# Wil-Lee/NN_BVH

Measured on AMD Instinct MI355X. Metric: Mray/s (closest-hit + any-hit), higher is better.
Workload: dtype f32; 1 GPU; crown, 1000x1400: one wavefront pass of 8 spp per step (8 spp per GPU-film) — primary, bounce-1 and bounce-2 closest-hit, shadow any-hit towards the light quads (batches pre-generated, hence independent: ONE launch; the dependent form is dependent_step), rays in --ray-order tile (a caller-side order the reference's integrator does not form: ray_order_probe), RecordShadowRayResult + RGBFilm::AddSam; sample_sets=4, geometry=procedural stand-in for crown (3548192 tris; data/crown.npz absent), tree=sah, triangles=3548192, nodes=7032259, rays_primary=11200000, rays_bounce=7410327, rays_bounce2=4392209, parallelism=tile-sharded x1, BVH replicated, film all-gather after the pass

## Files before the change

nn_bvh_amd/csrc/bvh_trace.hip:

```cpp
#include <hip/hip_runtime.h>
#include <stdint.h>

#include "bvh_trace.h"
#include "anim_math.h"
#include "spawn_math.h"
#include "trace_math.h"

namespace nnbvh {

constexpr int kDone = (int)0x80000000;
constexpr int kReturn = (int)0x80000001;
constexpr int kEnter = (int)0x80000002;

#ifndef NNBVH_MINW_CLOSEST
#define NNBVH_MINW_CLOSEST 6
#endif
#ifndef NNBVH_MINW_ANY
#define NNBVH_MINW_ANY 6
#endif
#ifndef NNBVH_LEAN_EXTRA_WAVES
#define NNBVH_LEAN_EXTRA_WAVES 2
#endif
#ifndef NNBVH_MINW_ALPHA
#define NNBVH_MINW_ALPHA 5
#endif
#ifndef NNBVH_MINW_ALPHA_PATCH
#define NNBVH_MINW_ALPHA_PATCH 3
#endif
#ifndef NNBVH_ANIM_ENTER_WEIGHT
#define NNBVH_ANIM_ENTER_WEIGHT 8
#endif
template <typename T>
__device__ __forceinline__ T pick_batch(const T (&a)[kMaxFusedBatches], int b) {
    static_assert(kMaxFusedBatches == 4, "written out for four batches");
    return b == 0 ? a[0] : (b == 1 ? a[1] : (b == 2 ? a[2] : a[3]));
}

template <int MODE, int W, int INST, int PATCH, int ALPHA = 0, int SOA = 0, int HOSTC = 0>
__global__ __launch_bounds__(kBlockThreads, (INST ? 1 : (ALPHA ? (ALPHA == 2 ? NNBVH_MINW_ALPHA_PATCH : NNBVH_MINW_ALPHA) : ((MODE == 0 || MODE == 3) ? NNBVH_MINW_CLOSEST : NNBVH_MINW_ANY) + (PATCH ? 0 : NNBVH_LEAN_EXTRA_WAVES))))
void trace_kernel(TraceParams p) {
    static_assert(PATCH || !INST, "two-level scenes need the ray direction");
    static_assert(PATCH || !ALPHA, "the alpha test hashes the ray direction");
    static_assert(!HOSTC || (PATCH && (MODE == 0 || MODE == 2 || (MODE == 3 && !ALPHA && W == 8)) && !SOA),
                  "candidate mode: general instances of modes 0 / 2 / 3");
    __shared__ float s_stack[kBlockThreads / 64][W][2][64];
    constexpr bool kLean = !PATCH && !INST;
    constexpr int kColdRi = 0, kColdD = 1, kColdHit = kLean ? 0 : (PATCH ? 4 : 1),
                  kColdHost = kColdHit + ((MODE == 0 || MODE == 3) ? 4 : 0);
    constexpr int kColdBase = kColdHost + (kLean ? 0 : 1);
    constexpr int kSaveO = kColdBase, kSaveInv = kColdBase + 3, kSaveShear = kColdBase + 6,
                  kSaveKz = kColdBase + 9, kSaveTmax = kColdBase + 10, kSaveD = kColdBase + 11,
                  kResume = kColdBase + 14, kCurInst = kColdBase + 15, kHitInst = kColdBase + 16,
                  kInnerHit = kColdBase + 17, kColdTime = kColdBase + 18, kPendSlot = kColdBase + 19;
    constexpr int kColdFields = kColdBase + (INST ? 20 : 0);
    __shared__ float s_cold[kBlockThreads / 64][kColdFields > 0 ? kColdFields : 1][64];

    const int lane = threadIdx.x & 63;
    const int wave = threadIdx.x >> 6;
    const int gtid = blockIdx.x * kBlockThreads + threadIdx.x;
    float(*stk)[2][64] = s_stack[wave];
    float(*cold)[64] = s_cold[wave];
    int riReg = -1;
    if (!kLean) cold[kColdRi][lane] = __int_as_float(-1);
    const long spillStride = (long)gridDim.x * kBlockThreads;

    int q = 0;
    if (p.nQueues > 1) {
        unsigned xcc;
        asm volatile("s_getreg_b32 %0, hwreg(HW_REG_XCC_ID)" : "=s"(xcc));
        q = (int)(xcc & 0xf) % p.nQueues;
    }
    int queuesTried = 0;
    int curBatch = 0;
    long nRays = p.n;
    if (p.nDev) {
        const long nd = (long)*p.nDev;
        nRays = nd < 0 ? 0 : (nd < nRays ? nd : nRays);
    }

#ifdef NNBVH_STATS
    unsigned long long st[16] = {0, 0, 0, 0, 0, 0, 0, 0, 0, 0, 0, 0, 0, 0, 0, 0};
    unsigned long long stPrev = __builtin_amdgcn_s_memtime();
    int stKind = 2;
#endif
    RayState r;
    RayMasks masks = {0ull, 0ull, 0ull, 0ull, 0ull, 0ull};
    float tMax = 0.0f;
    int visited = 0, tests = 0;
    int cur = kDone, sp = 0, base = 0;
    int floor = -1;
    bool found = false;
    bool exhausted = false;

    auto pop_entry = [&](int &ref, float &key) {
        --sp;
        ref = __float_as_int(stk[sp & (W - 1)][0][lane]);
        key = stk[sp & (W - 1)][1][lane];
        asm volatile("" : "+v"(ref), "+v"(key));
        if (sp < base) {
            const uint2 e = p.spill[(long)sp * spillStride + gtid];
            base = sp;
            ref = (int)e.x;
            key = __uint_as_float(e.y);
            asm volatile("" : "+v"(ref), "+v"(key));
        }
        if (MODE != 2) visited += 1;
    };
    auto pop_next = [&]() -> int {
        const int lowest = (INST && floor > 0) ? floor : 0;
        const int none = (INST && floor >= 0) ? kReturn : kDone;
        if (sp <= lowest) return none;
        int ref;
        float key;
        pop_entry(ref, key);
        if (key < tMax) return ref;
        while (sp > lowest) {
            pop_entry(ref, key);
            if (key < tMax) return ref;
        }
        return none;
    };

    auto enter_instance = [&](int slot, unsigned flags, float4 s0, float4 s1, float4 s2) {
        const float4 s3 = p.prims[slot + 3], s4 = p.prims[slot + 4], s5 = p.prims[slot + 5];
        const V3 dOuter = {cold[kColdD][lane], cold[kColdD + 1][lane], cold[kColdD + 2][lane]};
        cold[kSaveO][lane] = r.o.x;
        cold[kSaveO + 1][lane] = r.o.y;
        cold[kSaveO + 2][lane] = r.o.z;
        cold[kSaveInv][lane] = r.inv.x;
        cold[kSaveInv + 1][lane] = r.inv.y;
        cold[kSaveInv + 2][lane] = r.inv.z;
        cold[kSaveShear][lane] = r.sx;
        cold[kSaveShear + 1][lane] = r.sy;
        cold[kSaveShear + 2][lane] = r.sz;
        cold[kSaveKz][lane] = __int_as_float(r.kz);
        cold[kSaveTmax][lane] = tMax;
        cold[kSaveD][lane] = dOuter.x;
        cold[kSaveD + 1][lane] = dOuter.y;
        cold[kSaveD + 2][lane] = dOuter.z;
        cold[kResume][lane] = __int_as_float((flags & kPrimLast) ? kDone : ~(slot + 6));
        cold[kCurInst][lane] = __int_as_float(__float_as_int(s0.w) + 1);
        cold[kInnerHit][lane] = 0.0f;
        V3 oIn, dIn;
        float4 m0 = s2, m1 = s3, m2 = s4;
        if (INST == 2 && (flags & kPrimAnimated) && p.anim)
            anim_inverse_rows(p.anim + (long)kAnimStride * __float_as_int(s0.w), cold[kColdTime][lane], m0, m1, m2);
        apply_inverse_ray(m0, m1, m2, r.o, dOuter, tMax, oIn, dIn);
        r.o = oIn;
        cold[kColdD][lane] = dIn.x;
        cold[kColdD + 1][lane] = dIn.y;
        cold[kColdD + 2][lane] = dIn.z;
        r.inv = {1.0f / dIn.x, 1.0f / dIn.y, 1.0f / dIn.z};
        ray_shear(r, dIn);
        floor = sp;
        if (MODE != 2) visited += 1;
        float tEntry;
        const bool rootHit =
            slab_partial(s0.x, s0.y, s0.z, s1.x, s1.y, s1.z, r, tEntry) && (tEntry < tMax);
        cur = rootHit ? __float_as_int(s5.x) : kReturn;
    };

    auto leave_instance = [&]() {
        const bool innerHit = cold[kInnerHit][lane] != 0.0f;
        r.o = {cold[kSaveO][lane], cold[kSaveO + 1][lane], cold[kSaveO + 2][lane]};
        r.inv = {cold[kSaveInv][lane], cold[kSaveInv + 1][lane], cold[kSaveInv + 2][lane]};
        r.sx = cold[kSaveShear][lane];
        r.sy = cold[kSaveShear + 1][lane];
        r.sz = cold[kSaveShear + 2][lane];
        r.kz = __float_as_int(cold[kSaveKz][lane]);
        cold[kColdD][lane] = cold[kSaveD][lane];
        cold[kColdD + 1][lane] = cold[kSaveD + 1][lane];
        cold[kColdD + 2][lane] = cold[kSaveD + 2][lane];
        if (!innerHit) tMax = cold[kSaveTmax][lane];
        cold[kCurInst][lane] = 0.0f;
        floor = -1;
        const int resume = __float_as_int(cold[kResume][lane]);
        cur = (resume == kDone) ? pop_next() : resume;
    };

    auto prim_math = [&](const int slot, const float4 s0, const float4 s1, const float4 s2) {
        const unsigned flags = __float_as_uint(s1.w);
        if (INST && (flags & kPrimInstance)) {
            if (INST == 2 && NNBVH_ANIM_ENTER_WEIGHT > 0 && (flags & kPrimAnimated) && p.anim) {
                cold[kPendSlot][lane] = __int_as_float(slot);
                cur = kEnter;
            } else {
                enter_instance(slot, flags, s0, s1, s2);
            }
        } else if (!kLean && (flags & kPrimHost)) {
            if constexpr (HOSTC) {
                const int c = __float_as_int(cold[kColdHost][lane]);
                if (c >= 0) {
                    long ray = __float_as_int(cold[kColdRi][lane]);
                    int cap = p.hcCap;
                    int32_t *hcPrim = p.hcPrim, *hcInst = p.hcInst;
                    if constexpr (MODE == 3) {
                        const int b = (int)(ray >> kFusedIndexBits);
                        ray &= (1 << kFusedIndexBits) - 1;
                        cap = pick_batch(p.bHcCap, b);
                        hcPrim = pick_batch(p.bHcPrim, b);
                        hcInst = pick_batch(p.bHcInst, b);
                    }
                    if (c < cap) {
                        const long at = ray * cap + c;
                        hcPrim[at] = __float_as_int(s0.w);
                        hcInst[at] = INST ? __float_as_int(cold[kCurInst][lane]) : 0;
                    }
                    cold[kColdHost][lane] = __int_as_float(c < cap ? c + 1 : -1);
                }
            } else {
                cold[kColdHost][lane] = 1.0f;
            }
            cur = (flags & kPrimLast) ? pop_next() : ~(slot + 3);
        } else {
            tests += 1;
            bool hit;
            float x0, x1, x2, th;
            int next;
            if (!PATCH || !(flags & kPrimPatch)) {
                hit = triangle_test(r, tMax, (flags & kPrimDegenerate) != 0,
                                    {s0.x, s0.y, s0.z}, {s1.x, s1.y, s1.z},
                                    {s2.x, s2.y, s2.z}, x0, x1, x2, th, kLean ? &masks : nullptr);
                next = slot + ((ALPHA && (flags & kPrimSmooth)) ? 6 : 3);
                if (ALPHA && hit && (flags & kPrimAlpha)) {
                    const float a = s2.w;
                    if (a < 1) {
                        const V3 rd = {cold[kColdD][lane], cold[kColdD + 1][lane],
                                       cold[kColdD + 2][lane]};
                        const float u = (a <= 0) ? 1.f : hash_float_6f(r.o, rd);
                        if (u > a) {
                            hit = false;
                            RayState rn = r;
                            if (flags & kPrimSmooth) {
                                const float4 m0 = p.prims[slot + 3], m1 = p.prims[slot + 4], m2 = p.prims[slot + 5];
                                rn.o = alpha_retrace_origin({s0.x, s0.y, s0.z}, {s1.x, s1.y, s1.z}, {s2.x, s2.y, s2.z}, x0,
                                                            x1, x2, (flags & kPrimFlipN) != 0, rd, true, {m0.x, m0.y, m0.z},
                                                            {m1.x, m1.y, m1.z}, {m2.x, m2.y, m2.z});
                            } else {
                                rn.o = alpha_retrace_origin({s0.x, s0.y, s0.z}, {s1.x, s1.y, s1.z},
                                                            {s2.x, s2.y, s2.z}, x0, x1, x2,
                                                            (flags & kPrimFlipN) != 0, rd);
                            }
                            tests += 1;
                            float y0, y1, y2, tn;
                            if (triangle_test(rn, tMax - th, (flags & kPrimDegenerate) != 0,
                                              {s0.x, s0.y, s0.z}, {s1.x, s1.y, s1.z},
                                              {s2.x, s2.y, s2.z}, y0, y1, y2, tn))
                                cold[kColdHost][lane] = HOSTC ? __int_as_float(-2) : 1.0f;
                        }
                    }
                }
            } else {
                const float4 s3 = p.prims[slot + 3];
                x2 = 0.0f;
                const V3 rd = {cold[PATCH ? kColdD : 0][lane], cold[PATCH ? kColdD + 1 : 0][lane],
                               cold[PATCH ? kColdD + 2 : 0][lane]};
                next = slot + 4 + ((ALPHA == 2 && (flags & kPrimSmooth)) ? 4 : 0) + ((ALPHA == 2 && (flags & kPrimUV)) ? 2 : 0);
                if constexpr (ALPHA == 2) {
                    constexpr int kAlphaPatchDepth = 3;
                    const float a = (flags & kPrimAlpha) ? s2.w : 1.0f;
                    RayState rn = r;
                    float tm = tMax, t0 = 0.0f, t1 = 0.0f, t2 = 0.0f;
                    int k = 0;
                    for (;;) {
                        hit = patch_test(rn, rd, tm, {s0.x, s0.y, s0.z}, {s1.x, s1.y, s1.z}, {s2.x, s2.y, s2.z},
                                         {s3.x, s3.y, s3.z}, x0, x1, th);
                        if (!hit || !(a < 1)) break;
                        const float u = (a <= 0) ? 1.f : hash_float_6f(rn.o, rd);
                        if (!(u > a)) break;
                        if (k == kAlphaPatchDepth) {
                            hit = false;
                            cold[kColdHost][lane] = HOSTC ? __int_as_float(-2) : 1.0f;
                            break;
                        }
                        if (k == 0) t0 = th;
                        else if (k == 1) t1 = th;
                        else t2 = th;
                        ++k;
                        rn.o = patch_retrace_origin({s0.x, s0.y, s0.z}, {s1.x, s1.y, s1.z}, {s2.x, s2.y, s2.z},
                                                    {s3.x, s3.y, s3.z}, x0, x1, (flags & kPrimFlipN) != 0, rd,
                                                    (flags & kPrimSmooth) != 0, (flags & kPrimUV) != 0,
                                                    p.prims + slot + 4);
                        tm = tm - th;
                        tests += 1;
                    }
                    if (hit && k > 0) {
                        if (k == 3) th = th + t2;
                        if (k >= 2) th = th + t1;
                        th = th + t0;
                    }
                } else {
                    hit = patch_test(r, rd, tMax, {s0.x, s0.y, s0.z}, {s1.x, s1.y, s1.z},
                                     {s2.x, s2.y, s2.z}, {s3.x, s3.y, s3.z}, x0, x1, th);
                }
            }
            bool closestLane = MODE == 0;
            if (MODE == 3 && hit)
                closestLane = !((p.anyMask >> ((kLean ? riReg : __float_as_int(cold[kColdRi][lane])) >> kFusedIndexBits)) & 1u);
            if (hit) {
                if (closestLane) {
                    cold[kColdHit][lane] = s0.w;
                    cold[kColdHit + 1][lane] = x0;
                    cold[kColdHit + 2][lane] = x1;
                    cold[kColdHit + 3][lane] = x2;
                    tMax = th;
                    if (INST) {
                        cold[kHitInst][lane] = cold[kCurInst][lane];
                        cold[kInnerHit][lane] = 1.0f;
                    }
                    if constexpr (HOSTC && MODE == 0) {
                        const int c = __float_as_int(cold[kColdHost][lane]);
                        if (c > 0) p.hcBefore[__float_as_int(cold[kColdRi][lane])] = c;
                    }
                    if constexpr (HOSTC && MODE == 3) {
                        const int c = __float_as_int(cold[kColdHost][lane]);
                        if (c > 0) {
                            const int tag = __float_as_int(cold[kColdRi][lane]);
                            pick_batch(p.bHcBefore, tag >> kFusedIndexBits)[tag & ((1 << kFusedIndexBits) - 1)] = c;
                        }
                    }
                } else {
                    found = true;
                }
            }
            if (MODE != 0 && found) cur = kDone;
            else if (flags & kPrimLast) cur = pop_next();
            else cur = ~next;
        }
    };

    auto interior_math = [&](const float4 q0, const float4 q1, const float4 q2, const float4 q3) {
        const int ref0 = __float_as_int(q3.x), ref1 = __float_as_int(q3.y);
        const int axis = __float_as_int(q3.z);
        const bool swap = ((r.kz >> axis) & 1) != 0;
        const float k0 = kLean ? slab_entry_key(q0.x, q0.y, q0.z, q0.w, q1.x, q1.y, r, masks)
                               : slab_entry_key(q0.x, q0.y, q0.z, q0.w, q1.x, q1.y, r);
        const float k1 = kLean ? slab_entry_key(q1.z, q1.w, q2.x, q2.y, q2.z, q2.w, r, masks)
                               : slab_entry_key(q1.z, q1.w, q2.x, q2.y, q2.z, q2.w, r);
        const int nearRef = swap ? ref1 : ref0, farRef = swap ? ref0 : ref1;
        const float nearT = swap ? k1 : k0, farT = swap ? k0 : k1;
        visited += 1;
        const bool doPush = (MODE == 1) || (farT < __builtin_inff());
        if (doPush && sp - base == W - 1) {
            uint2 e;
            e.x = __float_as_uint(stk[base & (W - 1)][0][lane]);
            e.y = __float_as_uint(stk[base & (W - 1)][1][lane]);
            p.spill[(long)base * spillStride + gtid] = e;
            ++base;
        }
        stk[sp & (W - 1)][0][lane] = __int_as_float(farRef);
        stk[sp & (W - 1)][1][lane] = farT;
        sp += doPush ? 1 : 0;
        if (MODE == 0 || MODE == 3) visited += doPush ? 0 : 1;
        cur = nearT < tMax ? nearRef : pop_next();
    };
    auto interior_step = [&]() {
#ifdef NNBVH_STATS
        st[14] += 1;
        st[15] += __popcll(__ballot(cur >= 0));
#endif
        if (cur >= 0) {
            const float4 *rec = kLean ? reinterpret_cast<const float4 *>(reinterpret_cast<const char *>(p.wide) + ((unsigned)cur << 6))
                                      : p.wide + 4 * (long)cur;
            const float4 q3 = rec[3];
            const float4 q0 = rec[0], q1 = rec[1], q2 = rec[2];
            interior_math(q0, q1, q2, q3);
        }
    };

    for (;;) {
#ifdef NNBVH_STATS
        {
            const unsigned long long now = __builtin_amdgcn_s_memtime();
            st[10 + stKind] += now - stPrev;
            stPrev = now;
        }
#endif
        const bool isInt = cur >= 0;
        const bool isIdle = cur == kDone;
        const int nInt = __popcll(__ballot(isInt));
        const unsigned long long idleMask = __ballot(isIdle);
        const int nIdle = __popcll(idleMask);
        const int nEnter = (INST == 2 && NNBVH_ANIM_ENTER_WEIGHT > 0) ? __popcll(__ballot(cur == kEnter)) : 0;
        const int nPrim = 64 - nInt - nIdle - nEnter;

        const int sI = nInt * 16, sP = nPrim * p.primWeight;
        const int sR = exhausted ? 0 : nIdle * p.refillWeight;
#ifdef NNBVH_STATS
        unsigned long long &stTrips = (nIdle == 64 || (sR > sI && sR > sP)) ? st[4]
                                      : ((sP > sI || nInt == 0) ? st[2] : st[0]);
        (&stTrips)[0] += 1;
        (&stTrips)[1] += (nIdle == 64 || (sR > sI && sR > sP)) ? nIdle
                         : ((sP > sI || nInt == 0) ? nPrim : nInt);
        stKind = (&stTrips == &st[4]) ? 2 : ((&stTrips == &st[2]) ? 1 : 0);
        if (&stTrips == &st[0]) {
            st[6] += nInt;
            st[7] += nPrim;
            st[8] += nIdle;
        }
#endif
        if (nIdle == 64 || (sR > sI && sR > sP)) {
            const int ri = isIdle ? (kLean ? riReg : __float_as_int(cold[kColdRi][lane])) : -1;
            if constexpr (MODE == 3 && HOSTC) {
                if (ri >= 0) {
                    const int b = ri >> kFusedIndexBits;
                    const long idx = ri & ((1 << kFusedIndexBits) - 1);
                    void *outp = pick_batch(p.bOut, b);
                    const int c = __float_as_int(cold[kColdHost][lane]);
                    if (pick_batch(p.bHcCap, b) > 0) pick_batch(p.bHcCount, b)[idx] = c;
                    if ((p.anyMask >> b) & 1u) {
                        reinterpret_cast<uint8_t *>(outp)[idx] = found ? 1 : (c != 0 ? 2 : 0);
                    } else {
                        float4 h0, h1;
                        h0.x = cold[kColdHit][lane];
                        h0.y = tMax;
                        h0.z = cold[kColdHit + 1][lane];
                        h0.w = cold[kColdHit + 2][lane];
                        h1.x = cold[kColdHit + 3][lane];
                        h1.y = __int_as_float(visited);
                        h1.z = __int_as_float(tests);
                        h1.w = INST ? cold[kHitInst][lane] : 0.0f;
                        if (c < 0) h1.w = __int_as_float(-1);
                        float4 *out = reinterpret_cast<float4 *>(outp) + 2 * idx;
                        out[0] = h0;
                        out[1] = h1;
                    }
                }
            } else if (MODE == 3 && ri >= 0) {
                const int b = ri >> kFusedIndexBits;
                const long idx = ri & ((1 << kFusedIndexBits) - 1);
                void *outp = b == 0 ? p.bOut[0] : (b == 1 ? p.bOut[1] : (b == 2 ? p.bOut[2] : p.bOut[3]));
                const bool needHost = !kLean && p.hasHostPrims && cold[kColdHost][lane] != 0.0f;
                if ((p.anyMask >> b) & 1u) {
                    reinterpret_cast<uint8_t *>(outp)[idx] = found ? 1 : (needHost ? 2 : 0);
                } else {
                    float4 h0, h1;
                    h0.x = cold[kColdHit][lane];
                    h0.y = tMax;
                    h0.z = cold[kColdHit + 1][lane];
                    h0.w = cold[kColdHit + 2][lane];
                    h1.x = cold[kColdHit + 3][lane];
                    h1.y = __int_as_float(visited);
                    h1.z = __int_as_float(tests);
                    h1.w = INST ? cold[kHitInst][lane] : 0.0f;
                    if (needHost) h1.w = __int_as_float(-1);
                    float4 *out = reinterpret_cast<float4 *>(outp) + 2 * idx;
                    out[0] = h0;
                    out[1] = h1;
                }
            } else if (ri >= 0) {
                if (MODE == 0) {
                    float4 h0, h1;
                    h0.x = cold[kColdHit][lane];
                    h0.y = tMax;
                    h0.z = cold[kColdHit + 1][lane];
                    h0.w = cold[kColdHit + 2][lane];
                    h1.x = cold[kColdHit + 3][lane];
                    h1.y = __int_as_float(visited);
                    h1.z = __int_as_float(tests);
                    h1.w = INST ? cold[kHitInst][lane] : 0.0f;
                    if constexpr (HOSTC) {
                        const int c = __float_as_int(cold[kColdHost][lane]);
                        if (c < 0) h1.w = __int_as_float(-1);
                        p.hcCount[ri] = c;
                    } else if (!kLean && p.hasHostPrims && cold[kColdHost][lane] != 0.0f) {
                        h1.w = __int_as_float(-1);
                    }
                    float4 *out = reinterpret_cast<float4 *>(p.hits) + 2 * (long)ri;
                    out[0] = h0;
                    out[1] = h1;
                } else {
                    bool needHost;
                    if constexpr (HOSTC) {
                        const int c = __float_as_int(cold[kColdHost][lane]);
                        needHost = c != 0;
                        p.hcCount[ri] = c;
                    } else {
                        needHost = !kLean && p.hasHostPrims && cold[kColdHost][lane] != 0.0f;
                    }
                    p.occluded[ri] = found ? 1 : (needHost ? 2 : 0);
                    if (MODE == 1) {
                        if (p.visitedOut) p.visitedOut[ri] = visited;
                        if (p.testsOut) p.testsOut[ri] = tests;
                    }
                }
            }
            int newRi = -1;
            if (exhausted) break;
            long start = 0;
            for (;;) {
                if (MODE == 3) {
                    nRays = p.bN[curBatch];
                    if (const int32_t *nd = p.bNDev[curBatch]) {
                        const long v = *nd;
                        nRays = v < 0 ? 0 : (v < nRays ? v : nRays);
                    }
                }
                static_assert(kMaxQueues == 8, "queue ranges are computed with a shift by 3");
                const int qShift = p.nQueues > 1 ? 3 : 0;
                const long qBegin = (nRays * q) >> qShift, qEnd = (nRays * (q + 1)) >> qShift;
                unsigned got = 0;
                if (lane == 0)
                    got = atomicAdd(&p.queue[((MODE == 3 ? curBatch * p.nQueues : 0) + q) * kQueueStrideWords],
                                    (unsigned)nIdle);
                got = __builtin_amdgcn_readfirstlane(got);
                start = qBegin + (long)got;
                if (start < qEnd) {
                    const int rank = __builtin_amdgcn_mbcnt_hi(
                        (unsigned)(idleMask >> 32),
                        __builtin_amdgcn_mbcnt_lo((unsigned)idleMask, 0u));
                    if (isIdle && start + rank < qEnd) newRi = (int)(start + rank);
                    break;
                }
                if (++queuesTried >= p.nQueues) {
                    if (MODE == 3 && curBatch + 1 < p.nBatches) {
                        ++curBatch;
                        queuesTried = 0;
                        continue;
                    }
                    exhausted = true;
                    break;
                }
                q = (q + 1 == p.nQueues) ? 0 : q + 1;
            }
            if (isIdle) {
                const int tag = (MODE == 3 && newRi >= 0) ? (newRi | (curBatch << kFusedIndexBits)) : newRi;
                if (kLean) riReg = tag;
                else cold[kColdRi][lane] = __int_as_float(tag);
            }
            if (newRi >= 0) {
                const nnbvh_ray *batchRays = MODE == 3 ? p.bRays[curBatch] : p.rays;
                float4 r0, r1;
                if (!SOA || batchRays) {
                    const float4 *in = reinterpret_cast<const float4 *>(batchRays) + 2 * (long)newRi;
                    r0 = in[0];
                    r1 = in[1];
                } else {
                    const nnbvh_ray_soa &q = MODE == 3 ? p.bSoa[curBatch] : p.soa;
                    r0 = {q.ox[newRi], q.oy[newRi], q.oz[newRi], q.tmax ? q.tmax[newRi] : __builtin_inff()};
                    r1 = {q.dx[newRi], q.dy[newRi], q.dz[newRi], q.time ? q.time[newRi] : 0.0f};
                }
                r.o = {r0.x, r0.y, r0.z};
                tMax = r0.w;
                const V3 d = {r1.x, r1.y, r1.z};
                if (PATCH) {
                    cold[kColdD][lane] = d.x;
                    cold[kColdD + 1][lane] = d.y;
                    cold[kColdD + 2][lane] = d.z;
                }
                r.inv = {1.0f / d.x, 1.0f / d.y, 1.0f / d.z};
                ray_shear(r, d);
                if (MODE == 0 || MODE == 3) {
                    cold[kColdHit][lane] = __int_as_float(-1);
                    cold[kColdHit + 1][lane] = 0.0f;
                    cold[kColdHit + 2][lane] = 0.0f;
                    cold[kColdHit + 3][lane] = 0.0f;
                }
                if (INST) {
                    cold[kHitInst][lane] = 0.0f;
                    cold[kCurInst][lane] = 0.0f;
                    cold[kColdTime][lane] = r1.w;
                    floor = -1;
                }
                if (!kLean && (HOSTC || p.hasHostPrims)) cold[kColdHost][lane] = 0.0f;
                visited = 1;
                tests = 0;
                found = false;
                sp = base = 0;
                float tEntry;
                const bool rootHit =
                    slab_partial(p.rootMin[0], p.rootMin[1], p.rootMin[2], p.rootMax[0],
                                 p.rootMax[1], p.rootMax[2], r, tEntry) &&
                    (tEntry < tMax);
                cur = rootHit ? p.rootRef : kDone;
            }
            if (kLean) masks = ray_masks(r);
            continue;
        }

        if (INST == 2 && NNBVH_ANIM_ENTER_WEIGHT > 0 && nEnter > 0 &&
            ((nInt == 0 && nPrim == 0) || (nEnter * NNBVH_ANIM_ENTER_WEIGHT > sI && nEnter * NNBVH_ANIM_ENTER_WEIGHT > sP))) {
            if (cur == kEnter) {
                const int slot = __float_as_int(cold[kPendSlot][lane]);
                const float4 s0 = p.prims[slot], s1 = p.prims[slot + 1], s2 = p.prims[slot + 2];
                enter_instance(slot, __float_as_uint(s1.w), s0, s1, s2);
            }
            continue;
        }

        if (sP > sI || nInt == 0) {
            const int nPrep = (MODE == 3) ? 1 : p.primRepeat;
            int prep = 0;
            do {
            if (cur < 0 && cur != kDone) {
                if (INST && cur == kReturn) leave_instance();
                if (cur < 0 && cur != kDone && cur != kReturn && (INST != 2 || cur != kEnter)) {
                    const int slot = ~cur;
                    const float4 *pr = kLean ? reinterpret_cast<const float4 *>(reinterpret_cast<const char *>(p.prims) + ((unsigned)slot << 4))
                                             : p.prims + slot;
                    float4 s0 = pr[0], s1 = pr[1], s2 = pr[2];
                    asm volatile("" : "+v"(s0.x), "+v"(s0.y), "+v"(s0.z), "+v"(s0.w), "+v"(s1.x), "+v"(s1.y),
                                      "+v"(s1.z), "+v"(s1.w), "+v"(s2.x), "+v"(s2.y), "+v"(s2.z), "+v"(s2.w));
                    prim_math(slot, s0, s1, s2);
                }
            }
            } while (++prep < nPrep && __ballot(cur < 0 && cur != kDone) != 0ull);
        } else {
            if (MODE == 3) {
                interior_step();
                if (p.intRepeat > 1 && __ballot(cur >= 0) != 0ull) {
                    interior_step();
                    if (p.intRepeat > 2 && __ballot(cur >= 0) != 0ull) {
                        interior_step();
                        for (int rep = 3; rep < p.intRepeat && __ballot(cur >= 0) != 0ull; ++rep) interior_step();
                    }
                }
            } else {
            int rep = 0;
            do {
                interior_step();
            } while (++rep < p.intRepeat && __ballot(cur >= 0) != 0ull);
            }
        }
    }
#ifdef NNBVH_STATS
    if (lane == 0 && p.stats)
        for (int k = 0; k < 16; ++k) atomicAdd(&p.stats[k], st[k]);
#endif
}

template <int MODE, int W, int INST, int PATCH, int ALPHA = 0, int SOA = 0, int HOSTC = 0>
static hipError_t launch_one(const TraceParams &p, int blocks, hipStream_t stream, int *occupancy) {
    if (occupancy) {
        return hipOccupancyMaxActiveBlocksPerMultiprocessor(
            occupancy, trace_kernel<MODE, W, INST, PATCH, ALPHA, SOA, HOSTC>, kBlockThreads, 0);
    }
    hipLaunchKernelGGL((trace_kernel<MODE, W, INST, PATCH, ALPHA, SOA, HOSTC>), dim3((unsigned)blocks),
                       dim3(kBlockThreads), 0, stream, p);
    return hipGetLastError();
}

template <int MODE, int ALPHA, int HOSTC>
static hipError_t launch_inst(const TraceParams &p, int instanced, int blocks, hipStream_t stream, int *occupancy) {
    if (!instanced) return launch_one<MODE, 8, 0, 1, ALPHA, 0, HOSTC>(p, blocks, stream, occupancy);
    return p.anim ? launch_one<MODE, 8, 2, 1, ALPHA, 0, HOSTC>(p, blocks, stream, occupancy)
                  : launch_one<MODE, 8, 1, 1, ALPHA, 0, HOSTC>(p, blocks, stream, occupancy);
}
template <int MODE, int HOSTC>
static hipError_t launch_general(const TraceParams &p, int instanced, int patches, int blocks, hipStream_t stream,
                                 int *occupancy) {
    if (patches & 4) return launch_inst<MODE, 2, HOSTC>(p, instanced, blocks, stream, occupancy);
    if (patches & 2) return launch_inst<MODE, 1, HOSTC>(p, instanced, blocks, stream, occupancy);
    return launch_inst<MODE, 0, HOSTC>(p, instanced, blocks, stream, occupancy);
}

static hipError_t launch_fused(const TraceParams &p, int window, int instanced, int patches, int blocks,
                               hipStream_t stream, int *occupancy) {
    if (window != 8 || (patches & 2)) return hipErrorInvalidValue;
    if (p.hcCap > 0) {
        if (instanced) return p.anim ? launch_one<3, 8, 2, 1, 0, 0, 1>(p, blocks, stream, occupancy)
                                     : launch_one<3, 8, 1, 1, 0, 0, 1>(p, blocks, stream, occupancy);
        return launch_one<3, 8, 0, 1, 0, 0, 1>(p, blocks, stream, occupancy);
    }
    if (instanced) return p.anim ? launch_one<3, 8, 2, 1>(p, blocks, stream, occupancy)
                                 : launch_one<3, 8, 1, 1>(p, blocks, stream, occupancy);
    bool soa = false;
    for (int b = 0; b < p.nBatches; ++b) soa = soa || !p.bRays[b];
    if (!patches && !p.hasHostPrims && p.fits32)
        return soa ? launch_one<3, 8, 0, 0, 0, 1>(p, blocks, stream, occupancy) : launch_one<3, 8, 0, 0>(p, blocks, stream, occupancy);
    if (soa) return hipErrorInvalidValue;
    return launch_one<3, 8, 0, 1>(p, blocks, stream, occupancy);
}

template <int MODE>
static hipError_t launch_mode(const TraceParams &p, int window, int instanced, int patches, int blocks,
                              hipStream_t stream, int *occupancy) {
    if constexpr (MODE == 0 || MODE == 2) {
        if (p.hcCap > 0) return launch_general<MODE, 1>(p, instanced, patches, blocks, stream, occupancy);
    }
    if (instanced || (patches & 6)) return launch_general<MODE, 0>(p, instanced, patches, blocks, stream, occupancy);
    const bool soa = !p.rays && !occupancy;
    if (!patches && !p.hasHostPrims && p.fits32 && window == 8 && !instanced) {
        if (soa && MODE != 1) return launch_one<MODE == 1 ? 0 : MODE, 8, 0, 0, 0, 1>(p, blocks, stream, occupancy);
        if (!soa) return launch_one<MODE, 8, 0, 0>(p, blocks, stream, occupancy);
    }
    if (soa) return hipErrorInvalidValue;
    switch (window) {
    case 4: return launch_one<MODE, 4, 0, 1>(p, blocks, stream, occupancy);
    case 8: return launch_one<MODE, 8, 0, 1>(p, blocks, stream, occupancy);
    case 16: return launch_one<MODE, 16, 0, 1>(p, blocks, stream, occupancy);
    default: return hipErrorInvalidValue;
    }
}

__global__ void zero_queue_kernel(unsigned *queue, int words) {
    for (int i = threadIdx.x; i < words; i += blockDim.x) queue[i] = 0u;
}
hipError_t launch_zero_queue(unsigned *queue, int words, hipStream_t stream) {
    hipLaunchKernelGGL(zero_queue_kernel, dim3(1), dim3(256), 0, stream, queue, words);
    return hipGetLastError();
}

__global__ void zero_words_kernel(int32_t *words, long n) {
    for (long i = (long)blockIdx.x * blockDim.x + threadIdx.x; i < n; i += (long)gridDim.x * blockDim.x) words[i] = 0;
}
hipError_t launch_zero_words(int32_t *words, long n, int maxBlocks, hipStream_t stream) {
    long blocks = (n + 255) / 256;
    blocks = blocks < 1 ? 1 : (blocks < maxBlocks ? blocks : maxBlocks);
    hipLaunchKernelGGL(zero_words_kernel, dim3((unsigned)blocks), dim3(256), 0, stream, words, n);
    return hipGetLastError();
}

hipError_t launch_trace(int mode, const TraceParams &p, int window, int instanced, int patches, int blocks,
                        hipStream_t stream, int *occupancy) {
    switch (mode) {
    case 0: return launch_mode<0>(p, window, instanced, patches, blocks, stream, occupancy);
    case 1: return launch_mode<1>(p, window, instanced, patches, blocks, stream, occupancy);
    case 2: return launch_mode<2>(p, window, instanced, patches, blocks, stream, occupancy);
    case 3: return launch_fused(p, window, instanced, patches, blocks, stream, occupancy);
    default: return hipErrorInvalidValue;
    }
}

}
```

nn_bvh_amd/csrc/trace_math.h:

```cpp
#pragma once
#include <hip/hip_runtime.h>
#include <stdint.h>

namespace nnbvh {

#define DEV static __device__ __forceinline__

DEV constexpr float gamma_f(int n) {
    return ((float)n * 0x1p-24f) / (1.0f - (float)n * 0x1p-24f);
}

DEV float dop(float a, float b, float c, float d) {
    float cd = c * d;
    float diff = __builtin_fmaf(a, b, -cd);
    float err = __builtin_fmaf(-c, d, cd);
    return diff + err;
}

DEV float fmax3(float a, float b, float c) {
    return __builtin_fmaxf(__builtin_fmaxf(a, b), c);
}
DEV float max3(float a, float b, float c) {
    float m = a;
    if (m < b) m = b;
    if (m < c) m = c;
    return m;
}

struct V3 {
    float x, y, z;
};
DEV V3 cross(V3 v, V3 w) {
    return {dop(v.y, w.z, v.z, w.y), dop(v.z, w.x, v.x, w.z), dop(v.x, w.y, v.y, w.x)};
}
DEV float dot(V3 v, V3 w) { return v.x * w.x + v.y * w.y + v.z * w.z; }
DEV float len2(V3 v) { return v.x * v.x + v.y * v.y + v.z * v.z; }
DEV V3 sub(V3 a, V3 b) { return {a.x - b.x, a.y - b.y, a.z - b.z}; }
DEV float maxabs(V3 v) { return max3(__builtin_fabsf(v.x), __builtin_fabsf(v.y), __builtin_fabsf(v.z)); }
DEV float sel3(V3 v, int k) { return k == 0 ? v.x : (k == 1 ? v.y : v.z); }

struct RayState {
    V3 o, inv;
    float sx, sy, sz;
    int kz;
};

DEV void ray_shear(RayState &r, V3 d) {
    float ax = __builtin_fabsf(d.x), ay = __builtin_fabsf(d.y), az = __builtin_fabsf(d.z);
    int kz = (ax > ay) ? ((ax > az) ? 0 : 2) : ((ay > az) ? 1 : 2);
    int kx = kz + 1;
    if (kx == 3) kx = 0;
    int ky = kx + 1;
    if (ky == 3) ky = 0;
    float dx = kx == 0 ? d.x : (kx == 1 ? d.y : d.z);
    float dy = ky == 0 ? d.x : (ky == 1 ? d.y : d.z);
    float dz = kz == 0 ? d.x : (kz == 1 ? d.y : d.z);
    r.sx = -dx / dz;
    r.sy = -dy / dz;
    r.sz = 1.0f / dz;
    r.kz = (kz << 8) | (r.inv.x < 0.0f ? 1 : 0) | (r.inv.y < 0.0f ? 2 : 0) | (r.inv.z < 0.0f ? 4 : 0);
}

struct RayMasks {
    unsigned long long negX, negY, negZ;
    unsigned long long k0, k1, k2;
};
DEV RayMasks ray_masks(const RayState &r) {
    const int kz = r.kz >> 8;
    return {__ballot(r.inv.x < 0.0f), __ballot(r.inv.y < 0.0f), __ballot(r.inv.z < 0.0f),
            __ballot(kz == 0), __ballot(kz == 1), __ballot(kz == 2)};
}
DEV float sel_m(unsigned long long m, float a, float b) {
    float out;
    asm("v_cndmask_b32_e64 %0, %2, %1, %3" : "=v"(out) : "v"(a), "v"(b), "s"(m));
    return out;
}

DEV bool slab_partial(float mnx, float mny, float mnz, float mxx, float mxy, float mxz,
                      const RayState &r, float &tEntry) {
    constexpr float widen = 1.0f + 2.0f * gamma_f(3);
    float tMin = (((r.inv.x < 0.0f) ? mxx : mnx) - r.o.x) * r.inv.x;
    float tMax = (((r.inv.x < 0.0f) ? mnx : mxx) - r.o.x) * r.inv.x;
    float tyMin = (((r.inv.y < 0.0f) ? mxy : mny) - r.o.y) * r.inv.y;
    float tyMax = (((r.inv.y < 0.0f) ? mny : mxy) - r.o.y) * r.inv.y;
    tMax *= widen;
    tyMax *= widen;
    const bool out1 = (tMin > tyMax) | (tyMin > tMax);
    tMin = (tyMin > tMin) ? tyMin : tMin;
    tMax = (tyMax < tMax) ? tyMax : tMax;
    float tzMin = (((r.inv.z < 0.0f) ? mxz : mnz) - r.o.z) * r.inv.z;
    float tzMax = (((r.inv.z < 0.0f) ? mnz : mxz) - r.o.z) * r.inv.z;
    tzMax *= widen;
    const bool out2 = (tMin > tzMax) | (tzMin > tMax);
    tMin = (tzMin > tMin) ? tzMin : tMin;
    tMax = (tzMax < tMax) ? tzMax : tMax;
    tEntry = tMin;
    return !(out1 | out2) & (tMax > 0.0f);
}

DEV float slab_entry_key(float mnx, float mny, float mnz, float mxx, float mxy, float mxz, const RayState &r) {
    constexpr float widen = 1.0f + 2.0f * gamma_f(3);
    const float ax = (((r.inv.x < 0.0f) ? mxx : mnx) - r.o.x) * r.inv.x;
    const float bx = (((r.inv.x < 0.0f) ? mnx : mxx) - r.o.x) * r.inv.x;
    const float ay = (((r.inv.y < 0.0f) ? mxy : mny) - r.o.y) * r.inv.y;
    const float by = (((r.inv.y < 0.0f) ? mny : mxy) - r.o.y) * r.inv.y;
    const float az = (((r.inv.z < 0.0f) ? mxz : mnz) - r.o.z) * r.inv.z;
    const float bz = (((r.inv.z < 0.0f) ? mnz : mxz) - r.o.z) * r.inv.z;
    const float a = __builtin_fmaxf(__builtin_fmaxf(ax, ay), az);
    const float b = __builtin_fminf(__builtin_fminf(bx, by), bz) * widen;
    const bool ok = !__builtin_isunordered(ax, bx) & (a <= b) & (b > 0.0f);
    return ok ? a : __builtin_inff();
}

DEV float slab_entry_key(float mnx, float mny, float mnz, float mxx, float mxy, float mxz, const RayState &r,
                         const RayMasks &m) {
    constexpr float widen = 1.0f + 2.0f * gamma_f(3);
    const float ax = (sel_m(m.negX, mxx, mnx) - r.o.x) * r.inv.x;
    const float bx = (sel_m(m.negX, mnx, mxx) - r.o.x) * r.inv.x;
    const float ay = (sel_m(m.negY, mxy, mny) - r.o.y) * r.inv.y;
    const float by = (sel_m(m.negY, mny, mxy) - r.o.y) * r.inv.y;
    const float az = (sel_m(m.negZ, mxz, mnz) - r.o.z) * r.inv.z;
    const float bz = (sel_m(m.negZ, mnz, mxz) - r.o.z) * r.inv.z;
    const float a = __builtin_fmaxf(__builtin_fmaxf(ax, ay), az);
    const float b = __builtin_fminf(__builtin_fminf(bx, by), bz) * widen;
    const bool ok = !__builtin_isunordered(ax, bx) & (a <= b) & (b > 0.0f);
    return ok ? a : __builtin_inff();
}

DEV bool triangle_test(const RayState &r, float tMax, bool degenerate, V3 p0, V3 p1, V3 p2,
                       float &b0, float &b1, float &b2, float &tHit, const RayMasks *m = nullptr) {
    if (degenerate) return false;
    V3 a = sub(p0, r.o), b = sub(p1, r.o), c = sub(p2, r.o);
    float p0x, p0y, p0z, p1x, p1y, p1z, p2x, p2y, p2z;
    if (m) {
        auto px = [&](V3 v) { return sel_m(m->k2, v.x, sel_m(m->k0, v.y, v.z)); };
        auto py = [&](V3 v) { return sel_m(m->k1, v.x, sel_m(m->k2, v.y, v.z)); };
        auto pz = [&](V3 v) { return sel_m(m->k0, v.x, sel_m(m->k1, v.y, v.z)); };
        p0x = px(a), p0y = py(a), p0z = pz(a);
        p1x = px(b), p1y = py(b), p1z = pz(b);
        p2x = px(c), p2y = py(c), p2z = pz(c);
    } else {
        const int kz = r.kz >> 8;
        int kx = kz + 1;
        if (kx == 3) kx = 0;
        int ky = kx + 1;
        if (ky == 3) ky = 0;
        p0x = sel3(a, kx), p0y = sel3(a, ky), p0z = sel3(a, kz);
        p1x = sel3(b, kx), p1y = sel3(b, ky), p1z = sel3(b, kz);
        p2x = sel3(c, kx), p2y = sel3(c, ky), p2z = sel3(c, kz);
    }
    const float sx = r.sx, sy = r.sy, sz = r.sz;
    p0x += sx * p0z;
    p0y += sy * p0z;
    p1x += sx * p1z;
    p1y += sy * p1z;
    p2x += sx * p2z;
    p2y += sy * p2z;
    float e0 = dop(p1x, p2y, p1y, p2x);
    float e1 = dop(p2x, p0y, p2y, p0x);
    float e2 = dop(p0x, p1y, p0y, p1x);
    if (e0 == 0.0f || e1 == 0.0f || e2 == 0.0f) {
        double p2txp1ty = (double)p2x * (double)p1y;
        double p2typ1tx = (double)p2y * (double)p1x;
        e0 = (float)(p2typ1tx - p2txp1ty);
        double p0txp2ty = (double)p0x * (double)p2y;
        double p0typ2tx = (double)p0y * (double)p2x;
        e1 = (float)(p0typ2tx - p0txp2ty);
        double p1txp0ty = (double)p1x * (double)p0y;
        double p1typ0tx = (double)p1y * (double)p0x;
        e2 = (float)(p1typ0tx - p1txp0ty);
    }
    if ((e0 < 0 || e1 < 0 || e2 < 0) && (e0 > 0 || e1 > 0 || e2 > 0)) return false;
    float det = e0 + e1 + e2;
    if (det == 0) return false;
    p0z *= sz;
    p1z *= sz;
    p2z *= sz;
    float tScaled = e0 * p0z + e1 * p1z + e2 * p2z;
    if (det < 0 && (tScaled >= 0 || tScaled < tMax * det)) return false;
    else if (det > 0 && (tScaled <= 0 || tScaled > tMax * det)) return false;
    float invDet = 1.0f / det;
    float t = tScaled * invDet;
    const bool firstIsNan = __builtin_isunordered(p0z, p0x) | __builtin_isunordered(p0y, e0);
    float maxZt = fmax3(__builtin_fabsf(p0z), __builtin_fabsf(p1z), __builtin_fabsf(p2z));
    float deltaZ = gamma_f(3) * maxZt;
    float maxXt = fmax3(__builtin_fabsf(p0x), __builtin_fabsf(p1x), __builtin_fabsf(p2x));
    float maxYt = fmax3(__builtin_fabsf(p0y), __builtin_fabsf(p1y), __builtin_fabsf(p2y));
    float deltaX = gamma_f(5) * (maxXt + maxZt);
    float deltaY = gamma_f(5) * (maxYt + maxZt);
    float deltaE = 2.0f * (gamma_f(2) * maxXt * maxYt + deltaY * maxXt + deltaX * maxYt);
    float maxE = fmax3(__builtin_fabsf(e0), __builtin_fabsf(e1), __builtin_fabsf(e2));
    float deltaT = 3.0f * (gamma_f(3) * maxE * maxZt + deltaE * maxZt + deltaZ * maxE) *
                   __builtin_fabsf(invDet);
    if (!firstIsNan & (t <= deltaT)) return false;
    b0 = e0 * invDet;
    b1 = e1 * invDet;
    b2 = e2 * invDet;
    tHit = t;
    return true;
}

DEV bool quadratic(float a, float b, float c, float &t0, float &t1) {
    if (a == 0) {
        if (b == 0) return false;
        t0 = t1 = -c / b;
        return true;
    }
    float discrim = dop(b, b, 4.0f * a, c);
    if (discrim < 0) return false;
    float root = __builtin_sqrtf(discrim);
    float q = -0.5f * (b + __builtin_copysignf(root, b));
    t0 = q / a;
    t1 = c / q;
    if (t0 > t1) {
        float s = t0;
        t0 = t1;
        t1 = s;
    }
    return true;
}

DEV float det3(V3 r0, V3 r1, V3 r2) {
    float minor12 = dop(r1.y, r2.z, r1.z, r2.y);
    float minor02 = dop(r1.x, r2.z, r1.z, r2.x);
    float minor01 = dop(r1.x, r2.y, r1.y, r2.x);
    return __builtin_fmaf(r0.z, minor01, dop(r0.x, minor12, r0.y, minor02));
}

DEV V3 lerp3(float t, V3 a, V3 b) {
    float omt = 1.0f - t;
    return {omt * a.x + t * b.x, omt * a.y + t * b.y, omt * a.z + t * b.z};
}

DEV void patch_root(float u, const RayState &r, V3 rd, V3 p00, V3 p10, V3 p01, V3 p11, float &vnum,
                    float &tnum, float &p2) {
    V3 uo = lerp3(u, p00, p10);
    V3 ud = sub(lerp3(u, p01, p11), uo);
    V3 deltao = sub(uo, r.o);
    V3 perp = cross(rd, ud);
    p2 = len2(perp);
    vnum = det3({deltao.x, rd.x, perp.x}, {deltao.y, rd.y, perp.y}, {deltao.z, rd.z, perp.z});
    tnum = det3({deltao.x, ud.x, perp.x}, {deltao.y, ud.y, perp.y}, {deltao.z, ud.z, perp.z});
}

DEV bool patch_test(const RayState &r, V3 rd, float tMax, V3 p00, V3 p10, V3 p01, V3 p11, float &uOut,
                    float &vOut, float &tOut) {
    float a = dot(cross(sub(p10, p00), sub(p01, p11)), rd);
    float c = dot(cross(sub(p00, r.o), rd), sub(p01, p00));
    float b = dot(cross(sub(p10, r.o), rd), sub(p11, p10)) - (a + c);
    float u1, u2;
    if (!quadratic(a, b, c, u1, u2)) return false;
    float eps = gamma_f(10) * (maxabs(r.o) + maxabs(rd) + maxabs(p00) + maxabs(p10) +
                               maxabs(p01) + maxabs(p11));
    float t = tMax, u = 0.0f, v = 0.0f;
    if (0 <= u1 && u1 <= 1) {
        float v1, t1, p2;
        patch_root(u1, r, rd, p00, p10, p01, p11, v1, t1, p2);
        if (t1 > p2 * eps && 0 <= v1 && v1 <= p2) {
            u = u1;
            v = v1 / p2;
            t = t1 / p2;
        }
    }
    if (0 <= u2 && u2 <= 1 && u2 != u1) {
        float v2, t2, p2;
        patch_root(u2, r, rd, p00, p10, p01, p11, v2, t2, p2);
        t2 /= p2;
        if (0 <= v2 && v2 <= p2 && t > t2 && t2 > eps) {
            t = t2;
            u = u2;
            v = v2 / p2;
        }
    }
    if (t >= tMax) return false;
    uOut = u;
    vOut = v;
    tOut = t;
    return true;
}

DEV float next_up(float v) {
    if (__builtin_isinf(v) && v > 0.f) return v;
    if (v == -0.f) v = 0.f;
    unsigned ui = __float_as_uint(v);
    if (v >= 0) ++ui;
    else --ui;
    return __uint_as_float(ui);
}
DEV float next_down(float v) {
    if (__builtin_isinf(v) && v < 0.f) return v;
    if (v == 0.f) v = -0.f;
    unsigned ui = __float_as_uint(v);
    if (v > 0) --ui;
    else ++ui;
    return __uint_as_float(ui);
}
struct Ivl {
    float lo, hi;
};
DEV Ivl ivl(float a, float b) { return {(b < a) ? b : a, (a < b) ? b : a}; }
DEV Ivl ivl_from_value_and_error(float v, float err) {
    if (err == 0) return {v, v};
    return {next_down(v + (-err)), next_up(v + err)};
}
DEV Ivl ivl_add_f(Ivl a, float f) { return ivl(next_down(a.lo + f), next_up(a.hi + f)); }
DEV Ivl ivl_div_f(Ivl i, float f) {
    if (f == 0) return ivl(-__builtin_inff(), __builtin_inff());
    if (f > 0) return ivl(next_down(i.lo / f), next_up(i.hi / f));
    return ivl(next_down(i.hi / f), next_up(i.lo / f));
}
DEV void apply_inverse_ray(float4 r0, float4 r1, float4 r2, V3 o, V3 d, float &tMax, V3 &oOut,
                           V3 &dOut) {
    constexpr float g3 = gamma_f(3);
    const float px = (r0.x * o.x + r0.y * o.y) + (r0.z * o.z + r0.w);
    const float py = (r1.x * o.x + r1.y * o.y) + (r1.z * o.z + r1.w);
    const float pz = (r2.x * o.x + r2.y * o.y) + (r2.z * o.z + r2.w);
    const float ex0 = g3 * (__builtin_fabsf(r0.x * o.x) + __builtin_fabsf(r0.y * o.y) + __builtin_fabsf(r0.z * o.z));
    const float ey0 = g3 * (__builtin_fabsf(r1.x * o.x) + __builtin_fabsf(r1.y * o.y) + __builtin_fabsf(r1.z * o.z));
    const float ez0 = g3 * (__builtin_fabsf(r2.x * o.x) + __builtin_fabsf(r2.y * o.y) + __builtin_fabsf(r2.z * o.z));
    const float wp = (0.f * o.x + 0.f * o.y) + (0.f * o.z + 1.f);
    Ivl xp = ivl_from_value_and_error(px, ex0), yp = ivl_from_value_and_error(py, ey0),
        zp = ivl_from_value_and_error(pz, ez0);
    if (!(wp == 1)) {
        xp = ivl_div_f(xp, wp);
        yp = ivl_div_f(yp, wp);
        zp = ivl_div_f(zp, wp);
    }
    const float dx = r0.x * d.x + r0.y * d.y + r0.z * d.z;
    const float dy = r1.x * d.x + r1.y * d.y + r1.z * d.z;
    const float dz = r2.x * d.x + r2.y * d.y + r2.z * d.z;
    const float len2 = dx * dx + dy * dy + dz * dz;
    if (len2 > 0) {
        const float ex = (xp.hi - xp.lo) / 2, ey = (yp.hi - yp.lo) / 2, ez = (zp.hi - zp.lo) / 2;
        const float dt = (__builtin_fabsf(dx) * ex + __builtin_fabsf(dy) * ey + __builtin_fabsf(dz) * ez) / len2;
        xp = ivl_add_f(xp, dx * dt);
        yp = ivl_add_f(yp, dy * dt);
        zp = ivl_add_f(zp, dz * dt);
        tMax -= dt;
    }
    oOut = {(xp.lo + xp.hi) / 2, (yp.lo + yp.hi) / 2, (zp.lo + zp.hi) / 2};
    dOut = {dx, dy, dz};
}

}
```

Measured before the change: 4688 Mray/s.

## Add order-free any-hit traversal with leaf stashing and skip key culling on pops

For lean any-hit modes, adds a separate interior traversal path that pushes only far children within tMax, and pops without checking the stored key in pure any-hit mode. It also stashes one pending leaf so interior nodes keep being processed before the leaf is tested, which aims to keep lanes doing uniform interior work. In the fused mode it tracks which lanes hold any-hit rays and uses the order-free path only when every interior lane is any-hit. Separately, ray_shear reuses the precomputed inverse direction instead of a second division. The cost is extra control flow and register state, and stale stack entries may be visited because pops no longer cull by key.

```diff
diff --git a/nn_bvh_amd/csrc/bvh_trace.hip b/nn_bvh_amd/csrc/bvh_trace.hip
--- a/nn_bvh_amd/csrc/bvh_trace.hip
+++ b/nn_bvh_amd/csrc/bvh_trace.hip
@@ -91,6 +91,9 @@
     int floor = -1;
     bool found = false;
     bool exhausted = false;
+    constexpr bool kOrderFree = kLean && (MODE == 2 || MODE == 3);
+    int stash = kDone;
+    unsigned long long anyLanes = 0ull;
 
     auto pop_entry = [&](int &ref, float &key) {
         --sp;
@@ -113,6 +116,7 @@
         int ref;
         float key;
         pop_entry(ref, key);
+        if (kOrderFree && MODE == 2) return ref;
         if (key < tMax) return ref;
         while (sp > lowest) {
             pop_entry(ref, key);
@@ -323,9 +327,19 @@
                     found = true;
                 }
             }
-            if (MODE != 0 && found) cur = kDone;
-            else if (flags & kPrimLast) cur = pop_next();
-            else cur = ~next;
+            if (MODE != 0 && found) {
+                cur = kDone;
+                if (kOrderFree) stash = kDone;
+            } else if (flags & kPrimLast) {
+                if (kOrderFree && stash != kDone) {
+                    cur = stash;
+                    stash = kDone;
+                } else {
+                    cur = pop_next();
+                }
+            } else {
+                cur = ~next;
+            }
         }
     };
 
@@ -354,17 +368,71 @@
         if (MODE == 0 || MODE == 3) visited += doPush ? 0 : 1;
         cur = nearT < tMax ? nearRef : pop_next();
     };
-    auto interior_step = [&]() {
+    auto interior_math_any = [&](const float4 q0, const float4 q1, const float4 q2, const float4 q3) {
+        const int ref0 = __float_as_int(q3.x), ref1 = __float_as_int(q3.y);
+        const int axis = __float_as_int(q3.z);
+        const bool swap = ((r.kz >> axis) & 1) != 0;
+        const float k0 = slab_entry_key(q0.x, q0.y, q0.z, q0.w, q1.x, q1.y, r, masks);
+        const float k1 = slab_entry_key(q1.z, q1.w, q2.x, q2.y, q2.z, q2.w, r, masks);
+        const int nearRef = swap ? ref1 : ref0, farRef = swap ? ref0 : ref1;
+        const float nearT = swap ? k1 : k0, farT = swap ? k0 : k1;
+        const bool doPush = farT < tMax;
+        if (doPush && sp - base == W - 1) {
+            uint2 e;
+            e.x = __float_as_uint(stk[base & (W - 1)][0][lane]);
+            e.y = __float_as_uint(stk[base & (W - 1)][1][lane]);
+            p.spill[(long)base * spillStride + gtid] = e;
+            ++base;
+        }
+        stk[sp & (W - 1)][0][lane] = __int_as_float(farRef);
+        stk[sp & (W - 1)][1][lane] = farT;
+        sp += doPush ? 1 : 0;
+        int next = nearT < tMax ? nearRef : kDone;
+        if (next < 0 && next != kDone && stash == kDone && sp > 0) {
+            stash = next;
+            next = kDone;
+        }
+        if (next == kDone) {
+            if (sp > 0) {
+                --sp;
+                next = __float_as_int(stk[sp & (W - 1)][0][lane]);
+                asm volatile("" : "+v"(next));
+                if (sp < base) {
+                    next = (int)p.spill[(long)sp * spillStride + gtid].x;
+                    base = sp;
+                    asm volatile("" : "+v"(next));
+                }
+            } else {
+                next = stash;
+                stash = kDone;
+            }
+        }
+        cur = next;
+    };
+    auto interior_step = [&](const bool anyStep, const bool heldBack) {
 #ifdef NNBVH_STATS
         st[14] += 1;
         st[15] += __popcll(__ballot(cur >= 0));
 #endif
+        if (kOrderFree && (MODE == 2 || anyStep)) {
+            if (cur >= 0) {
+                const float4 *rec = reinterpret_cast<const float4 *>(reinterpret_cast<const char *>(p.wide) + ((unsigned)cur << 6));
+                const float4 q3 = rec[3];
+                const float4 q0 = rec[0], q1 = rec[1], q2 = rec[2];
+                interior_math_any(q0, q1, q2, q3);
+            }
+            return;
+        }
         if (cur >= 0) {
             const float4 *rec = kLean ? reinterpret_cast<const float4 *>(reinterpret_cast<const char *>(p.wide) + ((unsigned)cur << 6))
                                       : p.wide + 4 * (long)cur;
             const float4 q3 = rec[3];
             const float4 q0 = rec[0], q1 = rec[1], q2 = rec[2];
             interior_math(q0, q1, q2, q3);
+            if (kOrderFree && MODE == 3 && heldBack && cur == kDone) {
+                cur = stash;
+                stash = kDone;
+            }
         }
     };
 
@@ -378,7 +446,8 @@
 #endif
         const bool isInt = cur >= 0;
         const bool isIdle = cur == kDone;
-        const int nInt = __popcll(__ballot(isInt));
+        const unsigned long long intMask = __ballot(isInt);
+        const int nInt = __popcll(intMask);
         const unsigned long long idleMask = __ballot(isIdle);
         const int nIdle = __popcll(idleMask);
         const int nEnter = (INST == 2 && NNBVH_ANIM_ENTER_WEIGHT > 0) ? __popcll(__ballot(cur == kEnter)) : 0;
@@ -549,7 +618,7 @@
                     cold[kColdD + 2][lane] = d.z;
                 }
                 r.inv = {1.0f / d.x, 1.0f / d.y, 1.0f / d.z};
-                ray_shear(r, d);
+                ray_shear(r, d, kLean);
                 if (MODE == 0 || MODE == 3) {
                     cold[kColdHit][lane] = __int_as_float(-1);
                     cold[kColdHit + 1][lane] = 0.0f;
@@ -566,6 +635,7 @@
                 visited = 1;
                 tests = 0;
                 found = false;
+                stash = kDone;
                 sp = base = 0;
                 float tEntry;
                 const bool rootHit =
@@ -575,6 +645,7 @@
                 cur = rootHit ? p.rootRef : kDone;
             }
             if (kLean) masks = ray_masks(r);
+            if (kOrderFree && MODE == 3) anyLanes = __ballot(riReg >= 0 && ((p.anyMask >> (riReg >> kFusedIndexBits)) & 1u) != 0u);
             continue;
         }
 
@@ -607,18 +678,20 @@
             } while (++prep < nPrep && __ballot(cur < 0 && cur != kDone) != 0ull);
         } else {
             if (MODE == 3) {
-                interior_step();
+                const bool anyStep = kOrderFree && (intMask & ~anyLanes) == 0ull;
+                const bool heldBack = kOrderFree && (intMask & anyLanes) != 0ull;
+                interior_step(anyStep, heldBack);
                 if (p.intRepeat > 1 && __ballot(cur >= 0) != 0ull) {
-                    interior_step();
+                    interior_step(anyStep, heldBack);
                     if (p.intRepeat > 2 && __ballot(cur >= 0) != 0ull) {
-                        interior_step();
-                        for (int rep = 3; rep < p.intRepeat && __ballot(cur >= 0) != 0ull; ++rep) interior_step();
+                        interior_step(anyStep, heldBack);
+                        for (int rep = 3; rep < p.intRepeat && __ballot(cur >= 0) != 0ull; ++rep) interior_step(anyStep, heldBack);
                     }
                 }
             } else {
             int rep = 0;
             do {
-                interior_step();
+                interior_step(true, false);
             } while (++rep < p.intRepeat && __ballot(cur >= 0) != 0ull);
             }
         }
diff --git a/nn_bvh_amd/csrc/trace_math.h b/nn_bvh_amd/csrc/trace_math.h
--- a/nn_bvh_amd/csrc/trace_math.h
+++ b/nn_bvh_amd/csrc/trace_math.h
@@ -45,7 +45,7 @@
     int kz;
 };
 
-DEV void ray_shear(RayState &r, V3 d) {
+DEV void ray_shear(RayState &r, V3 d, bool szFromInv = false) {
     float ax = __builtin_fabsf(d.x), ay = __builtin_fabsf(d.y), az = __builtin_fabsf(d.z);
     int kz = (ax > ay) ? ((ax > az) ? 0 : 2) : ((ay > az) ? 1 : 2);
     int kx = kz + 1;
@@ -57,7 +57,7 @@
     float dz = kz == 0 ? d.x : (kz == 1 ? d.y : d.z);
     r.sx = -dx / dz;
     r.sy = -dy / dz;
-    r.sz = 1.0f / dz;
+    r.sz = szFromInv ? sel3(r.inv, kz) : 1.0f / dz;
     r.kz = (kz << 8) | (r.inv.x < 0.0f ? 1 : 0) | (r.inv.y < 0.0f ? 2 : 0) | (r.inv.z < 0.0f ? 4 : 0);
 }
 
```

After: 4583 Mray/s. 0.978x the previous value.
